# DecaYale/SYN3R

Measured on AMD Instinct MI355X. Metric: llff_3view_train_loop_iters_per_sec, higher is better.
Workload: dtype f32 raster / f16 UNet (f32 accumulate); 1 GPU; LLFF fern-like 3-view block: 50 raster fwd+bwd iters (l1 loss) (200000 Gaussians, 1920x1080, SH3) + 1 SVD (step,pass): CFG UNet fwd [2,14,8,72,128] f16 + fused Euler step; frames=14, parallelism=scene-parallel x1

## Files before the change

### include/syn3r_hip.h

```cpp
#ifndef SYN3R_HIP_H
#define SYN3R_HIP_H

#include <stddef.h>
#include <stdint.h>

#ifdef __cplusplus
extern "C" {
#endif

#define SYN3R_OK 0
#define SYN3R_E_INVALID (-1)
#define SYN3R_E_WORKSPACE (-2)
#define SYN3R_E_HIP (-3)

#define SYN3R_F32 0
#define SYN3R_F16 1

const char* syn3r_last_error(void);
int syn3r_version(void);
const char* syn3r_arch(void);

int syn3r_trace_enable(int on);
void* syn3r_trace_session(void);
int syn3r_trace_attach(void* session);
// ... 109 lines not shown
                                int W, int* radii, void* geom, size_t geom_bytes, long long* num_rendered_host,
                                int raw, int flags, const float* filter3d, void* stream);
int syn3r_raster_backward_f3d(int N, int sh_degree, int sh_coeffs, long long P, const float* means3D,
                              const float* scales, const float* rotations, const float* opacities, const float* shs,
                              const float* confidence, float scale_modifier, const float* viewmatrix,
                              const float* projmatrix, const float* campos, float tanfovx, float tanfovy, int H, int W,
                              const float* bg, const int* radii, void* geom, size_t geom_bytes,
                              const unsigned* point_list, void* image, size_t image_bytes, const float* dL_dcolor,
                              const float* dL_ddepth, const float* dL_dalpha, float* dL_dmeans3D, float* dL_dscales,
                              float* dL_drotations, float* dL_dopacities, float* dL_dshs, float* dL_dmeans2D,
                              float* dL_dconfidence, void* workspace, size_t workspace_bytes, int raw, int flags,
                              const float* filter3d, void* stream);
int syn3r_raster_backward_abs(int N, int sh_degree, int sh_coeffs, long long P, const float* means3D,
                              const float* scales, const float* rotations, const float* opacities, const float* shs,
                              const float* confidence, float scale_modifier, const float* viewmatrix,
                              const float* projmatrix, const float* campos, float tanfovx, float tanfovy, int H, int W,
                              const float* bg, const int* radii, void* geom, size_t geom_bytes,
                              const unsigned* point_list, void* image, size_t image_bytes, const float* dL_dcolor,
                              const float* dL_ddepth, const float* dL_dalpha, float* dL_dmeans3D, float* dL_dscales,
                              float* dL_drotations, float* dL_dopacities, float* dL_dshs, float* dL_dmeans2D,
                              float* dL_dconfidence, void* workspace, size_t workspace_bytes, int raw, int flags,
                              const float* filter3d, float* dL_dmeans2D_abs, void* stream);
size_t syn3r_raster_backward_cam_workspace_bytes(int N);
int syn3r_raster_backward_cam(int N, int sh_degree, int sh_coeffs, long long P, const float* means3D,
                              const float* scales, const float* rotations, const float* opacities, const float* shs,
                              const float* confidence, float scale_modifier, const float* viewmatrix,
                              const float* projmatrix, const float* campos, float tanfovx, float tanfovy, int H, int W,
                              const float* bg, const int* radii, void* geom, size_t geom_bytes,
                              const unsigned* point_list, void* image, size_t image_bytes, const float* dL_dcolor,
                              const float* dL_ddepth, const float* dL_dalpha, float* dL_dmeans3D, float* dL_dscales,
                              float* dL_drotations, float* dL_dopacities, float* dL_dshs, float* dL_dmeans2D,
                              float* dL_dconfidence, void* workspace, size_t workspace_bytes, int raw, int flags,
                              const float* filter3d, float* dL_dmeans2D_abs, float* dL_dcamera, int accumulate,
                              void* stream);

size_t syn3r_sort_pairs_workspace_bytes(long long n);
int syn3r_sort_pairs(unsigned long long* keys, unsigned* vals, unsigned long long* keys_tmp, unsigned* vals_tmp,
                     long long n, int nbits, void* workspace, size_t workspace_bytes, int* result_in_tmp,
                     void* stream);


int syn3r_gemm_f16(const void* A, long long lda, const void* W, void* out, long long ldc, const void* bias,
                   const void* rowvec, long long ldrv, int rows_per_vec, int rv_group_rows, const void* residual, long long ldr,
                   const void* aux, long long ldaux, float s_acc, float s_res, float s_aux, int M, int N, int K,
                   void* gn_partials, size_t gn_partials_bytes, int* gn_written, void* stream);

int syn3r_gemm_2src_supported(int M, int N, int K1, int K2, long long lda1, long long lda2);
int syn3r_gemm_2src_f16(const void* A1, long long lda1, int K1, const void* A2, long long lda2, int K2, const void* W,
                        void* out, long long ldc, const void* bias, int M, int N, void* gn_partials, size_t gn_partials_bytes,
                        int* gn_written, void* stream);

int syn3r_gemm_set_tile(int bm);

int syn3r_gemm_set_splitk_workspace(void* workspace, size_t bytes);

int syn3r_gemm_geglu_f16(const void* A, long long lda, const void* Wpacked, const void* bias_packed, void* out,
                         long long ldc, int M, int D, int K, void* stream);

size_t syn3r_feedforward_workspace_bytes(int M, int D);
int syn3r_feedforward_f16(const void* x, long long ldx, const void* w1_packed, const void* b1_packed, int D,
                          const void* w2, const void* b2, void* out, long long ldc, const void* residual,
                          long long ldr, const void* aux, long long ldaux, float s_acc, float s_res, float s_aux,
                          int M, int C_in, int C_out, void* workspace, size_t workspace_bytes, void* stream);

int syn3r_feedforward_p64_supported(int M, int D, int C_in);
int syn3r_feedforward_p64_f16(const void* x, long long ldx, const void* w1_packed64, const void* b1_packed64, int D,
                              const void* w2, const void* b2, void* out, long long ldc, const void* residual,
                              long long ldr, const void* aux, long long ldaux, float s_acc, float s_res, float s_aux,
                              int M, int C_in, int C_out, void* workspace, size_t workspace_bytes, void* stream);

int syn3r_feedforward_fused_f16(const void* x, long long ldx, const void* w1_chunked, const void* b1_chunked, int D,
                                const void* w2, const void* b2, void* out, long long ldc, const void* residual,
                                long long ldr, const void* aux, long long ldaux, float s_acc, float s_res, float s_aux,
                                int M, int C, void* stream);

int syn3r_feedforward_fused_ln_f16(const void* x, long long ldx, const void* ln_gamma, const void* ln_beta, float ln_eps,
                                   const void* w1_chunked, const void* b1_chunked, int D, const void* w2, const void* b2,
                                   void* out, long long ldc, const void* residual, long long ldr, const void* aux,
                                   long long ldaux, float s_acc, float s_res, float s_aux, int M, int C, void* stream);

int syn3r_feedforward_fused_addln_f16(const void* x, long long ldx, const void* addvec, int rows_per_vec, const void* ln_gamma,
                                      const void* ln_beta, float ln_eps, const void* w1_chunked, const void* b1_chunked, int D,
                                      const void* w2, const void* b2, void* out, long long ldc, const void* aux, long long ldaux,
                                      float s_acc, float s_res, float s_aux, int M, int C, void* stream);

int syn3r_layernorm_linear320_f16(const void* x, long long ldx, const void* ln_gamma, const void* ln_beta, float ln_eps,
                                  const void* W, void* out, long long ldc, int M, int N, int C, void* stream);

int syn3r_conv2d3x3_f16(const void* X, const void* W, void* out, long long ldc, const void* bias,
                        const void* rowvec, long long ldrv, int rows_per_vec, const void* residual, long long ldr,
                        float s_acc, float s_res, int NB, int Hi, int Wi, int Cin, int Cout, int stride, int upsample,
                        int pad_lo, void* gn_partials, size_t gn_partials_bytes, int* gn_written, void* stream);

int syn3r_pack_upsample4_f16(const void* w, void* w4, int Cout, int Cin);
int syn3r_conv2d3x3_up4_f16(const void* X, const void* w4, void* out, const void* bias, const void* residual, int NB, int Hi, int Wi,
                            int Cin, int Cout, void* gn_partials, size_t gn_partials_bytes, int* gn_written, void* stream);

int syn3r_tconv3_f16(const void* X, const void* W, void* out, long long ldc, const void* bias, const void* rowvec,
                     long long ldrv, int rows_per_vec, const void* residual, long long ldr, float s_acc, float s_res,
                     int B, int F, int HW, int Cin, int Cout, void* gn_partials, size_t gn_partials_bytes, int* gn_written,
                     void* stream);

int syn3r_attention_f16(const void* q, const void* k, const void* v, long long ld, void* out, long long ldo,
                        int nseq, int S, int heads, void* stream);

int syn3r_attention_temporal_f16(const void* q, const void* k, const void* v, long long ld, void* out,
// ... 161 lines not shown
```

### syn3r_amd/_lib.py

```python
from __future__ import annotations

import ctypes as C
from pathlib import Path

import torch

_LIB_PATH = Path(__file__).resolve().parent / "lib" / "libsyn3r_hip.so"
_lib = None

c_f = C.c_float
c_i = C.c_int
c_p = C.c_void_p
c_sz = C.c_size_t
c_ll = C.c_longlong
c_d = C.c_double

F32, F16 = 0, 1
RASTER_ANTIALIAS = 1

FILTER3D_VARIANCE, FILTER3D_NEAR, FILTER3D_MARGIN = 0.2, 0.2, 0.15

_SCENE = [c_p, c_p, c_p, c_p, c_p, c_p, c_f, c_p, c_p, c_p, c_f, c_f, c_i, c_i]
_RASTER_PREPROCESS = [c_i, c_i, c_i] + _SCENE + [c_p, c_p, c_sz, C.POINTER(c_ll)]
_RASTER_BACKWARD = ([c_i, c_i, c_i, c_ll] + _SCENE + [c_p, c_p, c_p, c_sz, c_p, c_p, c_sz]
# ... 2 lines not shown
_CAM = [c_i, c_i, c_p, c_p, c_p, c_i, c_p]
CAMERA_GRAD = 35

SIGNATURES = {
    "syn3r_last_error": (C.c_char_p, []),
    "syn3r_version": (c_i, []),
    "syn3r_arch": (C.c_char_p, []),
    "syn3r_trace_enable": (c_i, [c_i]),
    "syn3r_trace_filter": (c_i, [C.c_char_p]),
    "syn3r_trace_report": (c_i, [C.c_char_p, c_sz]),
    "syn3r_trace_session": (c_p, []),
    "syn3r_trace_attach": (c_i, [c_p]),
    "syn3r_inverse_warp_workspace_bytes": (c_sz, [c_i]),
    "syn3r_inverse_warp": (c_i, [c_p, c_p, c_p, c_p, c_p, c_p, c_p, c_f, c_i, c_i, c_i,
                                 c_p, c_p, c_p, c_p, c_p, c_p, c_p, c_p, c_p, c_p, c_p, c_p, c_sz, c_p]),
    "syn3r_reproj_error": (c_i, [c_p, c_p, c_p, c_p, c_p, c_p, c_p, c_i, c_i, c_p, c_p]),
    "syn3r_warp_post": (c_i, [c_p, c_p, c_p, c_i, c_i, c_i, c_i, c_i, c_p, c_p, c_p, c_p, c_p, c_p, c_p]),
    "syn3r_fuse_uncertainty": (c_i, [c_p, c_p, c_p, c_i, c_i, c_i, c_i, c_i, c_p, c_p, c_p, c_p]),
    "syn3r_forward_warp_workspace_bytes": (c_sz, [c_i, c_i]),
    "syn3r_forward_warp": (c_i, [c_p, c_p, c_p, c_p, c_p, c_p, c_i, c_i, c_p, c_p, c_p, c_p, c_sz, c_p]),
    "syn3r_step_workspace_bytes": (c_sz, [c_i, c_i, c_i, c_i]),
    "syn3r_step_interp": (c_i, [c_p, c_i, c_p, c_i, c_p, c_p, c_p, c_f, c_f, c_f, c_f, c_f, c_f, c_i,
                                c_p, c_p, c_p, c_i, c_i, c_i, c_i, c_p, c_sz, c_p]),
    "syn3r_step_replace": (c_i, [c_p, c_i, c_p, c_i, c_p, c_p, c_p, c_f, c_f, c_f, c_f,
                                 c_p, c_p, c_i, c_i, c_i, c_i, c_p, c_sz, c_p]),
    "syn3r_raster_geom_bytes": (c_sz, [c_i]),
    "syn3r_raster_image_bytes": (c_sz, [c_i, c_i]),
    "syn3r_raster_binning_bytes": (c_sz, [c_ll]),
    "syn3r_raster_preprocess": (c_i, _RASTER_PREPROCESS + _STREAM),
    "syn3r_raster_preprocess_raw": (c_i, _RASTER_PREPROCESS + _STREAM),
    "syn3r_raster_preprocess_ex": (c_i, _RASTER_PREPROCESS + _EX),
    "syn3r_raster_preprocess_f3d": (c_i, _RASTER_PREPROCESS + _F3D),
    "syn3r_raster_render": (c_i, [c_i, c_i, c_i, c_p, c_p, c_p, c_sz, c_p, c_sz, c_p, c_sz, c_ll, c_p, c_p, c_p,
                                  C.POINTER(c_p), c_p]),
    "syn3r_raster_backward_workspace_bytes": (c_sz, [c_i]),
    "syn3r_raster_backward": (c_i, _RASTER_BACKWARD + _STREAM),
    "syn3r_raster_backward_raw": (c_i, _RASTER_BACKWARD + _STREAM),
    "syn3r_raster_backward_ex": (c_i, _RASTER_BACKWARD + _EX),
    "syn3r_raster_backward_f3d": (c_i, _RASTER_BACKWARD + _F3D),
    "syn3r_raster_backward_abs": (c_i, _RASTER_BACKWARD + _ABS),
    "syn3r_raster_backward_cam_workspace_bytes": (c_sz, [c_i]),
    "syn3r_raster_backward_cam": (c_i, _RASTER_BACKWARD + _CAM),
    "syn3r_filter3d_workspace_bytes": (c_sz, [c_i]),
    "syn3r_filter3d_compute": (c_i, [c_p, c_i, c_p, c_i, c_f, c_f, c_f, c_p, c_p, c_sz, c_p]),
    "syn3r_sort_pairs_workspace_bytes": (c_sz, [c_ll]),
    "syn3r_sort_pairs": (c_i, [c_p, c_p, c_p, c_p, c_ll, c_i, c_p, c_sz, C.POINTER(c_i), c_p]),
    "syn3r_gaussian_activate": (c_i, [c_i, c_p, c_p, c_p, c_p, c_p, c_p, c_p]),
    "syn3r_gaussian_activate_backward": (c_i, [c_i, c_p, c_p, c_p, c_p, c_p, c_p, c_p, c_p, c_p, c_p, c_p]),
    "syn3r_densification_stats": (c_i, [c_i, c_p, c_p, c_p, c_p, c_p, c_p]),
    "syn3r_densification_stats_abs": (c_i, [c_i, c_p, c_p, c_p, c_p, c_p, c_p, c_p, c_p]),
    "syn3r_gemm_f16": (c_i, [c_p, c_ll, c_p, c_p, c_ll, c_p, c_p, c_ll, c_i, c_i, c_p, c_ll, c_p, c_ll, c_f, c_f, c_f,
                             c_i, c_i, c_i, c_p, c_sz, C.POINTER(c_i), c_p]),
    "syn3r_gemm_set_tile": (c_i, [c_i]),
    "syn3r_gemm_geglu_f16": (c_i, [c_p, c_ll, c_p, c_p, c_p, c_ll, c_i, c_i, c_i, c_p]),
    "syn3r_feedforward_workspace_bytes": (c_sz, [c_i, c_i]),
    "syn3r_feedforward_f16": (c_i, [c_p, c_ll, c_p, c_p, c_i, c_p, c_p, c_p, c_ll, c_p, c_ll, c_p, c_ll, c_f, c_f, c_f,
                                    c_i, c_i, c_i, c_p, c_sz, c_p]),
    "syn3r_feedforward_p64_f16": (c_i, [c_p, c_ll, c_p, c_p, c_i, c_p, c_p, c_p, c_ll, c_p, c_ll, c_p, c_ll, c_f, c_f, c_f,
                                    c_i, c_i, c_i, c_p, c_sz, c_p]),
    "syn3r_feedforward_p64_supported": (c_i, [c_i, c_i, c_i]),
    "syn3r_feedforward_fused_f16": (c_i, [c_p, c_ll, c_p, c_p, c_i, c_p, c_p, c_p, c_ll, c_p, c_ll, c_p, c_ll, c_f, c_f, c_f,
                                          c_i, c_i, c_p]),
    "syn3r_feedforward_fused_ln_f16": (c_i, [c_p, c_ll, c_p, c_p, c_f, c_p, c_p, c_i, c_p, c_p, c_p, c_ll, c_p, c_ll, c_p, c_ll,
                                             c_f, c_f, c_f, c_i, c_i, c_p]),
    "syn3r_feedforward_fused_addln_f16": (c_i, [c_p, c_ll, c_p, c_i, c_p, c_p, c_f, c_p, c_p, c_i, c_p, c_p, c_p, c_ll, c_p, c_ll,
                                                c_f, c_f, c_f, c_i, c_i, c_p]),
    "syn3r_layernorm_linear320_f16": (c_i, [c_p, c_ll, c_p, c_p, c_f, c_p, c_p, c_ll, c_i, c_i, c_i, c_p]),
    "syn3r_conv2d3x3_f16": (c_i, [c_p, c_p, c_p, c_ll, c_p, c_p, c_ll, c_i, c_p, c_ll, c_f, c_f,
                                  c_i, c_i, c_i, c_i, c_i, c_i, c_i, c_i, c_p, c_sz, C.POINTER(c_i), c_p]),
    "syn3r_pack_upsample4_f16": (c_i, [c_p, c_p, c_i, c_i]),
    "syn3r_conv2d3x3_up4_f16": (c_i, [c_p, c_p, c_p, c_p, c_p, c_i, c_i, c_i, c_i, c_i, c_p, c_sz, C.POINTER(c_i), c_p]),
    "syn3r_tconv3_f16": (c_i, [c_p, c_p, c_p, c_ll, c_p, c_p, c_ll, c_i, c_p, c_ll, c_f, c_f,
                               c_i, c_i, c_i, c_i, c_i, c_p, c_sz, C.POINTER(c_i), c_p]),
    "syn3r_attention_f16": (c_i, [c_p, c_p, c_p, c_ll, c_p, c_ll, c_i, c_i, c_i, c_p]),
    "syn3r_attention_temporal_f16": (c_i, [c_p, c_p, c_p, c_ll, c_p, c_ll, c_i, c_i, c_i, c_i, c_p]),
    "syn3r_groupnorm_workspace_bytes": (c_sz, [c_i, c_i]),
    "syn3r_groupnorm_f16": (c_i, [c_p, c_p, c_i, c_i, c_i, c_p, c_p, c_f, c_i, c_p, c_sz, c_p]),
    "syn3r_groupnorm_2src_f16": (c_i, [c_p, c_i, c_p, c_i, c_p, c_i, c_i, c_p, c_p, c_f, c_i, c_p, c_sz, c_p]),
    "syn3r_groupnorm_pre_f16": (c_i, [c_p, c_i, c_p, c_p, c_i, c_p, c_p, c_i, c_i, c_p, c_p, c_f, c_i, c_p, c_sz, c_p]),
    "syn3r_gn_partials_bytes": (c_sz, [c_i, c_i]),
    "syn3r_gemm_2src_supported": (c_i, [c_i, c_i, c_i, c_i, c_ll, c_ll]),
    "syn3r_gemm_2src_f16": (c_i, [c_p, c_ll, c_i, c_p, c_ll, c_i, c_p, c_p, c_ll, c_p, c_i, c_i, c_p, c_sz, C.POINTER(c_i), c_p]),
    "syn3r_layernorm_f16": (c_i, [c_p, c_p, c_p, c_p, c_i, c_ll, c_i, c_p, c_p, c_f, c_p]),
    "syn3r_geglu_f16": (c_i, [c_p, c_p, c_ll, c_i, c_p]),
    "syn3r_softmax_rows_f16": (c_i, [c_p, c_p, c_ll, c_i, c_ll, c_f, c_p]),
    "syn3r_time_conv_out": (c_i, [c_p, c_ll, c_p, c_p, c_p, c_i, c_i, c_ll, c_p]),
    "syn3r_l1_loss_workspace_bytes": (c_sz, [c_ll]),
    "syn3r_l1_loss": (c_i, [c_p, c_p, c_ll, c_f, c_p, c_p, c_sz, c_p]),
    "syn3r_l1_loss_backward": (c_i, [c_p, c_p, c_ll, c_f, c_p, c_p, c_p]),
    "syn3r_image_mse": (c_i, [c_p, c_p, c_ll, c_p, c_p, c_sz, c_p]),
    "syn3r_photo_loss_workspace_bytes": (c_sz, [c_i, c_i, c_i]),
    "syn3r_photo_loss": (c_i, [c_p, c_p, c_i, c_i, c_i, c_f, c_f, c_p, c_p, c_sz, c_p]),
    "syn3r_photo_loss_backward": (c_i, [c_p, c_p, c_i, c_i, c_i, c_f, c_f, c_p, c_p, c_p, c_p]),
    "syn3r_photo_loss_step": (c_i, [c_p, c_p, c_i, c_i, c_i, c_f, c_f, c_p, c_p, c_p, c_p, c_sz, c_p]),
    "syn3r_photo_loss_map_workspace_bytes": (c_sz, [c_i, c_i, c_i]),
    "syn3r_photo_loss_map": (c_i, [c_p, c_p, c_p, c_i, c_i, c_i, c_f, c_f, c_p, c_p, c_sz, c_p]),
    "syn3r_photo_loss_map_backward": (c_i, [c_p, c_p, c_p, c_i, c_i, c_i, c_f, c_f, c_p, c_p, c_p, c_p]),
    "syn3r_photo_loss_map_step": (c_i, [c_p, c_p, c_p, c_i, c_i, c_i, c_f, c_f, c_p, c_p, c_p, c_p, c_sz, c_p]),
    "syn3r_l1_loss_map": (c_i, [c_p, c_p, c_p, c_ll, c_ll, c_f, c_p, c_p, c_sz, c_p]),
    "syn3r_l1_loss_map_backward": (c_i, [c_p, c_p, c_p, c_ll, c_ll, c_f, c_p, c_p, c_p]),
    "syn3r_depth_corr_loss_workspace_bytes": (c_sz, [c_ll]),
    "syn3r_depth_corr_loss": (c_i, [c_p, c_p, c_ll, c_f, c_f, c_i, c_p, c_p, c_sz, c_p]),
    "syn3r_depth_corr_loss_backward": (c_i, [c_p, c_p, c_ll, c_f, c_f, c_i, c_p, c_p, c_sz, c_p, c_p]),
    "syn3r_depth_corr_loss_step": (c_i, [c_p, c_p, c_ll, c_f, c_f, c_i, c_p, c_p, c_p, c_p, c_sz, c_p]),
    "syn3r_exposure_apply": (c_i, [c_p, c_p, c_i, c_i, c_p, c_p]),
    "syn3r_exposure_backward_workspace_bytes": (c_sz, [c_i, c_i]),
# ... 174 lines not shown
```

### syn3r_amd/csrc/gemm.hip

```cpp
#include "common.h"
#include <cstdlib>
#include <algorithm>
#include <atomic>
#include <type_traits>

using namespace syn3r;

namespace {

#include "gemm_common.h"
#include "gemm_dma160.h"
#include "gemm_dma.h"
#include "gemm_wide.h"
#include "gemm_z.h"
#include "gemm_dmap.h"
#include "gemm_dmapd.h"
#include "gemm_g256.h"
#include "gemm_ffn.h"

int persistent_blocks() {
    static std::atomic<int> cus_of[64];
    static const int forced = tune_env("SYN3R_PERSISTENT_BLOCKS", 0);
    if (forced > 0) return forced < 8 ? 8 : forced;
    int dev = 0;
    if (hipGetDevice(&dev) != hipSuccess || dev < 0 || dev >= 64) dev = 0;
    int n = cus_of[dev].load(std::memory_order_relaxed);
    if (n == 0) {
        int v = 0;
        n = (hipDeviceGetAttribute(&v, hipDeviceAttributeMultiprocessorCount, dev) == hipSuccess && v > 0) ? v : 256;
        if (n < 8) n = 8;
        cus_of[dev].store(n, std::memory_order_relaxed);
    }
    return n;
}

size_t gn_partials_bytes(long long M, long long N) { return (size_t)(M / 32) * 2 * (size_t)(N / 10) * sizeof(float); }
int gn_request(GemmParams& p, void* buf, size_t bytes, const char* who) {
    SYN3R_REQUIRE((buf == nullptr) == (bytes == 0), "%s: gn_partials pointer and size must both be given or both be zero", who);
    SYN3R_REQUIRE(((uintptr_t)buf % 16) == 0, "%s: the gn_partials buffer must be 16-byte aligned", who);
    if (!buf || p.M % 32 != 0 || p.N % 80 != 0 || p.geglu_D > 0 || p.out_tiled || bytes < gn_partials_bytes(p.M, p.N)) return SYN3R_OK;
    p.gn_part = (float*)buf; p.gn_units = p.N / 10;
    return SYN3R_OK;
}

template <void (*KERNEL)(GemmParams)>
int launch_tiles(const char* family, size_t lds, long long grid, int block, hipStream_t stream, const GemmParams& q, int* gn_written,
                 const char* base, int b0 = 0, int b1 = 0) {
    static DevOnce once;
    if (int rc = set_max_lds(once, (const void*)KERNEL, (int)lds, family)) return rc;
    char name[96];
    if (trace_on()) {
        const int n = snprintf(name, sizeof(name), base, b0, b1);
        if (trace_detail()) snprintf(name + n, sizeof(name) - n, "[M%d,N%d,K%d,e%d]", q.M, q.N, q.K, q.geglu_D > 0 ? 2 : (q.residual != nullptr));
    }
    SYN3R_LAUNCH_NAMED(name, KERNEL, dim3((unsigned)grid), dim3(block), lds, stream, q);
    hipError_t e = hipGetLastError();
    if (e != hipSuccess) { set_error("%s launch: %s", family, hipGetErrorString(e)); return SYN3R_E_HIP; }
    if (gn_written) *gn_written = q.gn_part != nullptr;
    return SYN3R_OK;
}

long long wide_tiles(const GemmParams& p) { return (long long)((p.M + WBM - 1) / WBM) * ((p.N + WBN - 1) / WBN); }
bool wide_fills(const GemmParams& p) {
    const long long tiles = wide_tiles(p), rounds = (tiles + 255) / 256;
    return tiles * 10 >= rounds * 256 * 8;
}

int band_width(const GemmParams& p) {
    static const int band_env = tune_env("SYN3R_Z_BAND", 0);
    if (band_env > 0) return band_env;
// ... 155 lines not shown
    bool split = false;
    int rc = launch_splitk<MODE>(p, stream, &split);
    if (split || rc) return rc;
    int bm = g_dma_bm > 0 ? g_dma_bm : ((MODE != MODE_DENSE || tiles256(p) >= 256) ? 256 : 128);
    return bm == 128 ? launch_dma_bm<MODE, 128>(p, stream, gn_written) : launch_dma_bm<MODE, 256>(p, stream, gn_written);
}

int check_common(const GemmParams& p, const char* who) {
    SYN3R_REQUIRE(p.A && p.W && p.out, "%s: null operand", who);
    SYN3R_REQUIRE(SYN3R_DIM_OK(p.M) && SYN3R_DIM_OK(p.N) && SYN3R_DIM_OK(p.K), "%s: bad sizes M=%d N=%d K=%d", who, p.M, p.N, p.K);
    SYN3R_REQUIRE(p.K % BK == 0, "%s: K=%d must be a multiple of %d", who, p.K, BK);
    SYN3R_REQUIRE(p.ldc % 8 == 0 && p.ldc >= p.N, "%s: ldc=%lld must be >= N and a multiple of 8", who, p.ldc);
    SYN3R_REQUIRE(!p.residual || (p.ldr % 8 == 0 && p.ldr >= p.N), "%s: bad residual stride", who);
    SYN3R_REQUIRE(!p.aux || (p.ldaux % 8 == 0 && p.ldaux >= p.N), "%s: bad aux stride", who);
    SYN3R_REQUIRE(!p.rowvec || (p.rows_per_vec != 0 && p.ldrv >= p.N), "%s: bad rowvec arguments", who);
    SYN3R_REQUIRE(p.rv_group >= 0 && (p.rv_group == 0 || p.rows_per_vec < 0), "%s: rv_group_rows needs rows_per_vec < 0", who);
    SYN3R_REQUIRE(((uintptr_t)p.A | (uintptr_t)p.W | (uintptr_t)p.out | (uintptr_t)p.residual | (uintptr_t)p.aux) % 16 == 0,
                  "%s: operands must be 16-byte aligned", who);
    return SYN3R_OK;
}

int ffn_workspace_check(const char* who, const void* workspace, size_t workspace_bytes, size_t need) {
    if (!workspace || workspace_bytes < need) {
        set_error("%s: workspace %zu < %zu", who, workspace_bytes, need);
        return SYN3R_E_WORKSPACE;
    }
    SYN3R_REQUIRE((uintptr_t)workspace % 16 == 0, "%s: workspace must be 16-byte aligned", who);
    return SYN3R_OK;
}
int ffn_net2(const char* who, const void* hidden_tiled, int D, const void* w2, const void* b2, void* out, long long ldc, const void* residual,
             long long ldr, const void* aux, long long ldaux, float s_acc, float s_res, float s_aux, int M, int C_out, hipStream_t stream) {
    GemmParams q{};
    q.A = (const __half*)hidden_tiled; q.lda = D; q.a_tiled = 1; q.W = (const __half*)w2; q.out = (__half*)out; q.ldc = ldc;
    q.bias = (const __half*)b2; q.residual = (const __half*)residual; q.ldr = ldr; q.aux = (const __half*)aux; q.ldaux = ldaux;
    q.s_acc = s_acc; q.s_res = s_res; q.s_aux = s_aux; q.M = M; q.N = C_out; q.K = D;
    int rc = check_common(q, who);
    if (rc) return rc;
    return launch_dma<MODE_DENSE>(q, stream);
}

}

extern "C" int syn3r_gemm_set_splitk_workspace(void* workspace, size_t bytes) {
    SYN3R_REQUIRE((workspace == nullptr) == (bytes == 0), "gemm_set_splitk_workspace: pointer and size must both be given or both be zero");
    SYN3R_REQUIRE(((uintptr_t)workspace % 16) == 0, "gemm_set_splitk_workspace: the workspace must be 16-byte aligned");
    g_splitk_ws = workspace;
    g_splitk_bytes = bytes;
    return SYN3R_OK;
}

extern "C" size_t syn3r_gn_partials_bytes(int M, int N) {
    if (!SYN3R_DIM_OK(M) || !SYN3R_DIM_OK(N) || M % 32 != 0 || N % 80 != 0) return 0;
    return gn_partials_bytes(M, N);
}

extern "C" int syn3r_gemm_set_tile(int bm) {
    SYN3R_REQUIRE(bm == 0 || bm == -128 || bm == -256 || bm == -320 || bm == -322, "gemm_set_tile: bm must be 0, -128, -256, -320 or -322");
    g_dma_bm = (bm == -128 || bm == -256) ? -bm : bm;
    return SYN3R_OK;
}

extern "C" int syn3r_gemm_2src_supported(int M, int N, int K1, int K2, long long lda1, long long lda2) {
    if (M < 8 || N < 8 || M % 8 || N % 8 || K1 <= 0 || K2 <= 0 || K1 % BK || K2 % BK) return 0;
    if ((long long)M * lda1 >= (1ll << 31) || (long long)M * lda2 >= (1ll << 31) || (long long)N * (K1 + K2) >= (1ll << 31)) return 0;
    return 1;
}

constexpr int SKINNY_MAX_M = 16;
template <int MR>
__global__ void __launch_bounds__(256) k_gemm_skinny(GemmParams p) {
    const int lane = threadIdx.x & 63, wv = threadIdx.x >> 6;
    const int n0 = (blockIdx.x * 4 + wv) * 2;
    if (n0 >= p.N) return;
    const bool two = n0 + 1 < p.N;
    const __half* w0 = p.W + (long long)n0 * p.K;
    const __half* w1 = p.W + (long long)(two ? n0 + 1 : n0) * p.K;
    float acc0[MR], acc1[MR];
#pragma unroll
    for (int m = 0; m < MR; ++m) { acc0[m] = 0.f; acc1[m] = 0.f; }
    for (int k = lane * 8; k < p.K; k += 512) {
        const half8 a = *(const half8*)(w0 + k), b = *(const half8*)(w1 + k);
#pragma unroll
        for (int m = 0; m < MR; ++m) {
            if (m < p.M) {
                const half8 x = *(const half8*)(p.A + (long long)m * p.lda + k);
#pragma unroll
                for (int e = 0; e < 8; ++e) {
                    acc0[m] += (float)x[e] * (float)a[e];
                    acc1[m] += (float)x[e] * (float)b[e];
                }
            }
        }
    }
#pragma unroll
    for (int m = 0; m < MR; ++m) {
        if (m < p.M) {
            float s0 = wave_sum(acc0[m]), s1 = wave_sum(acc1[m]);
            if (lane == 0) {
                float b0 = p.bias ? __half2float(p.bias[n0]) : 0.f;
                p.out[(long long)m * p.ldc + n0] = __float2half((s0 + b0) * p.s_acc);
                if (two) {
                    float b1 = p.bias ? __half2float(p.bias[n0 + 1]) : 0.f;
                    p.out[(long long)m * p.ldc + n0 + 1] = __float2half((s1 + b1) * p.s_acc);
                }
            }
        }
// ... 329 lines not shown
```

### syn3r_amd/csrc/gemm_ffn.h

```cpp

constexpr int F_C = 320, F_HC = 64, F_BM = 128;
constexpr int F_X_BYTES = F_BM * F_C * 2;
constexpr int F_SLOT = 160 * BK * 2;

struct FfnParams {
    GemmParams e;
    const __half* w1;
    const __half* b1;
    int D;
    const __half* ln_g;
    const __half* ln_b;
    float ln_eps;
    const __half* ln_add;
    int ln_add_rpv;
};

typedef _Float16 half4v __attribute__((ext_vector_type(4)));
#define DS_READ64(dst, addr, OFF) asm volatile("ds_read_b64 %0, %1 offset:" #OFF : "=v"(dst) : "v"(addr))
#define DS_WRITE64(addr, val) asm volatile("ds_write_b64 %0, %1" ::"v"(addr), "v"(val) : "memory")

__device__ __forceinline__ void ln_tile320(char* smem_raw, int tid, int m0, int M, float cf, const __half* ln_g, const __half* ln_b,
                                           float ln_eps, const __half* add, int add_rpv) {
    {
        const int r = tid >> 2, part = tid & 3;
        const int f = (r >> 1) & 1;
        half8 xv[5][2], addv[5][2];
        if (add) {
            int m = m0 + r;
            m = m < M ? m : M - 1;
            const __half* av = add + (long long)(m / add_rpv) * F_C;
#pragma unroll
            for (int kt = 0; kt < 5; ++kt)
#pragma unroll
                for (int e = 0; e < 2; ++e) addv[kt][e] = *(const half8*)(av + (kt * 8 + part + 4 * (e ^ f)) * 8);
        }
        asm volatile("s_waitcnt vmcnt(0)" ::: "memory");
        __syncthreads();
#pragma unroll
        for (int kt = 0; kt < 5; ++kt)
#pragma unroll
            for (int e = 0; e < 2; ++e)
                xv[kt][e] = *(const half8*)(smem_raw + kt * 16384 + r * 128 + (((part + 4 * (e ^ f)) ^ (r & 7)) << 4));
        if (add) {
#pragma unroll
            for (int kt = 0; kt < 5; ++kt)
#pragma unroll
                for (int e = 0; e < 2; ++e) xv[kt][e] = xv[kt][e] + addv[kt][e];
        }
        float s0 = 0.f, s1 = 0.f;
#pragma unroll
        for (int kt = 0; kt < 5; ++kt)
#pragma unroll
            for (int i = 0; i < 8; ++i) { s0 += (float)xv[kt][0][i]; s1 += (float)xv[kt][1][i]; }
        const float sa = f ? s1 : s0, sb = f ? s0 : s1;
        float s = sa + sb;
        s += __shfl_xor(s, 2, 64);
        s += __shfl_xor(s, 1, 64);
        const float mean = s / cf;
        float q0 = 0.f, q1 = 0.f;
        {
#pragma clang fp contract(off)
#pragma unroll
            for (int kt = 0; kt < 5; ++kt)
#pragma unroll
                for (int i = 0; i < 8; ++i) {
                    const float da = (float)xv[kt][0][i] - mean, db = (float)xv[kt][1][i] - mean;
                    const float da2 = da * da, db2 = db * db;
                    q0 += da2; q1 += db2;
                }
        }
        const float qa = f ? q1 : q0, qb = f ? q0 : q1;
        float qq = qa + qb;
        qq += __shfl_xor(qq, 2, 64);
        qq += __shfl_xor(qq, 1, 64);
        const float rstd = rsqrtf(qq / cf + ln_eps);
#pragma unroll
        for (int kt = 0; kt < 5; ++kt)
#pragma unroll
            for (int e = 0; e < 2; ++e) {
                const int cv = kt * 8 + part + 4 * (e ^ f);
                const half8 g = *(const half8*)(ln_g + cv * 8), b = *(const half8*)(ln_b + cv * 8);
                half8 o;
#pragma unroll
                for (int i = 0; i < 8; ++i) o[i] = (_Float16)(((float)xv[kt][e][i] - mean) * rstd * (float)g[i] + (float)b[i]);
                *(half8*)(smem_raw + kt * 16384 + r * 128 + (((part + 4 * (e ^ f)) ^ (r & 7)) << 4)) = o;
            }
        __syncthreads();
    }

}

constexpr int R_SLOTS = 7;
constexpr int R_H = R_SLOTS * F_SLOT;
constexpr int R_BIAS = R_H + F_BM * F_HC * 2;
constexpr int R_LDS = R_BIAS + 8 * 512;

__global__ void __launch_bounds__(512, 2) k_ffn320r(FfnParams q) {
    const GemmParams& p = q.e;
    extern __shared__ __attribute__((aligned(16))) char smem_raw[];
    const int tid = threadIdx.x, lane = tid & 63;
    const int wv = __builtin_amdgcn_readfirstlane(tid >> 6);
    const int wm = wv >> 1, wn = wv & 1;
    const int tiles_m = (p.M + F_BM - 1) / F_BM;
    const int m0 = (int)xcd_remap(blockIdx.x, (unsigned)tiles_m) * F_BM;
    const int nchunks = q.D / F_HC;
    const long long D = q.D;
    const int fr = lane & 15, fq = lane >> 4;
    typedef _Float16 half4e __attribute__((ext_vector_type(4)));

    const int prow = lane >> 3;
    const int csrc = (lane & 7) ^ prow;
    const int nbw = wv < 4 ? 3 : 2;
    const int b_first = wv < 4 ? wv * 3 : 12 + (wv - 4) * 2;
    unsigned ow1 = (unsigned)((((wv * 2) * 8 + prow) * F_C + csrc * 8) * 2);
    unsigned ow2 = (unsigned)(((long long)(b_first * 8 + prow) * D + csrc * 8) * 2);
    unsigned ob1 = (unsigned)(lane * 4);
    char* const bias_line = smem_raw + R_BIAS + wv * 512;
    auto issue_w1 = [&](int ij, int ir) {
        asm volatile("" : "+v"(ow1), "+v"(ob1));
        long long soff = ((long long)ij * (128 * F_C) + ir * BK) * 2;
        asm volatile("" : "+s"(soff));
        const char* src = (const char*)q.w1 + soff;
        char* slot = smem_raw + ir * F_SLOT;
#pragma unroll
        for (int i = 0; i < 2; ++i)
            __builtin_amdgcn_global_load_lds((gbl_void_t*)(src + i * (8 * F_C * 2) + (size_t)ow1), (lds_void_t*)(slot + (wv * 2 + i) * 1024), 16, 0, 0);
        if (ir == 0) {
            long long boff = (long long)ij * 256;
            asm volatile("" : "+s"(boff));
            __builtin_amdgcn_global_load_lds((gbl_void_t*)((const char*)q.b1 + boff + (size_t)ob1), (lds_void_t*)(bias_line + (ij & 1) * 256), 4, 0, 0);
        }
    };
    auto issue_w2 = [&](int ij) {
        asm volatile("" : "+v"(ow2));
#pragma unroll
        for (int hh = 0; hh < 2; ++hh) {
            long long soff = ((long long)hh * 160 * D + (long long)ij * F_HC) * 2;
            asm volatile("" : "+s"(soff));
            const char* src = (const char*)p.W + soff;
            char* slot = smem_raw + (5 + hh) * F_SLOT;
// ... 250 lines not shown
                    half8 rr = res[it];
                    if (p.res_add) rr = rr + radd[it];
#pragma unroll
                    for (int e = 0; e < 8; ++e) f[e] += p.s_res * (float)rr[e];
                }
                if (p.aux) {
                    const half8 av = *(const half8*)(p.aux + (long long)m * p.ldaux + n);
#pragma unroll
                    for (int e = 0; e < 8; ++e) f[e] += p.s_aux * (float)av[e];
                }
#pragma unroll
                for (int e = 0; e < 8; ++e) v[e] = (_Float16)f[e];
            }
            *(half8*)(p.out + (long long)m * p.ldc + n) = v;
        }
    }
}

int launch_ffn320(const FfnParams& q, hipStream_t stream) {
    static DevOnce once;
    int rc = set_max_lds(once, (const void*)k_ffn320r, R_LDS, "hipFuncSetAttribute(ffn320r)");
    if (rc) return rc;
    const int tiles = (q.e.M + F_BM - 1) / F_BM;
    char name[96];
    if (trace_on()) {
        if (trace_detail()) snprintf(name, sizeof(name), "k_gemm_ffn320[M%d,D%d,e%d]", q.e.M, q.D, q.e.residual != nullptr);
        else snprintf(name, sizeof(name), "k_gemm_ffn320");
    }
    SYN3R_LAUNCH_NAMED(name, k_ffn320r, dim3(tiles), dim3(512), R_LDS, stream, q);
    SYN3R_LAUNCH_CHECK("ffn320r launch");
    return SYN3R_OK;
}

constexpr int Q_SLOT = F_C * 32 * 2;
constexpr int Q_RING = F_X_BYTES;
constexpr int Q_ST = Q_RING + 3 * Q_SLOT;
constexpr int Q_ST_WAVE = 16 * WN * 2;
constexpr int Q_LDS = Q_ST + 8 * Q_ST_WAVE;

struct LnLinParams {
    const __half* x; long long ldx;
    const __half* W;
    __half* out; long long ldc;
    int M, N, C;
    const __half* ln_g; const __half* ln_b; float ln_eps;
};

__global__ void __launch_bounds__(512, 2) k_lnlin320(LnLinParams p) {
    extern __shared__ __attribute__((aligned(16))) char smem_raw[];
    const int tid = threadIdx.x, lane = tid & 63;
    const int wv = __builtin_amdgcn_readfirstlane(tid >> 6);
    const int wm = wv >> 2, wn = wv & 3;
    const int tiles_m = (p.M + F_BM - 1) / F_BM;
    const int m0 = (int)xcd_remap(blockIdx.x, (unsigned)tiles_m) * F_BM;
    const int nstage = (p.N / F_C) * 10;
    const bool full = m0 + F_BM <= p.M;

    const int wprow = lane >> 2;
    const int wcsrc = (lane & 3) ^ h_swz(wprow);
    const int nbw = wv < 4 ? 3 : 2;
    const int b_first = wv < 4 ? wv * 3 : 12 + (wv - 4) * 2;
    const __half* w_lane = p.W + (long long)(b_first * 16 + wprow) * F_C + wcsrc * 8;
    char* const ring = smem_raw + Q_RING;
    int ig = 0, islot = 0;
    auto issue_next = [&]() {
        if (ig >= nstage) return;
        const int c = ig / 10, ks = ig - c * 10;
        const __half* src = w_lane + (long long)c * (F_C * F_C) + ks * 32;
        char* slot = ring + islot * Q_SLOT;
#pragma unroll
        for (int i = 0; i < 3; ++i)
            if (i < nbw)
                __builtin_amdgcn_global_load_lds((gbl_void_t*)(src + i * 16 * F_C), (lds_void_t*)(slot + (b_first + i) * 1024), 16, 0, 0);
        ++ig;
        if (++islot == 3) islot = 0;
    };

    {
        const int prow = lane >> 3;
        const int csrc = (lane & 7) ^ prow;
#pragma unroll
        for (int kt = 0; kt < 5; ++kt)
#pragma unroll
            for (int i = 0; i < 2; ++i) {
                int m = m0 + (wv * 2 + i) * 8 + prow;
                m = m < p.M ? m : p.M - 1;
                __builtin_amdgcn_global_load_lds((gbl_void_t*)(p.x + (long long)m * p.ldx + kt * BK + csrc * 8),
                                                 (lds_void_t*)(smem_raw + kt * 16384 + (wv * 2 + i) * 1024), 16, 0, 0);
            }
    }
    issue_next();
    issue_next();
    ln_tile320(smem_raw, tid, m0, p.M, (float)p.C, p.ln_g, p.ln_b, p.ln_eps, nullptr, 1);

    const int fr = lane & 15, fq = lane >> 4;
    const unsigned lds0 = (unsigned)(size_t)(__attribute__((address_space(3))) char*)smem_raw;
    const unsigned sw0 = (unsigned)(((0 + fq) ^ (fr & 7)) << 4), sw1 = (unsigned)(((4 + fq) ^ (fr & 7)) << 4);
    const unsigned x_row = lds0 + (unsigned)((wm * 64 + fr) * 128);
    const unsigned w_row = (unsigned)((wn * 80 + fr) * 64) + (unsigned)((fq ^ h_swz(fr)) << 4);
    const unsigned st_base = lds0 + Q_ST + (unsigned)(wv * Q_ST_WAVE);
    unsigned st_wr[TN];
#pragma unroll
    for (int j = 0; j < TN; ++j) st_wr[j] = st_base + (unsigned)(fr * (WN * 2) + ((j * 2 + (fq >> 1) + fr) % 10) * 16 + (fq & 1) * 8);
    int st_col[3];
#pragma unroll
    for (int it = 0; it < 3; ++it) {
        const int q = lane + it * 64, row = q / (WN / 8), chp = q - row * (WN / 8);
        st_col[it] = ((chp + 20 - row) % 10) * 8;
    }
    typedef _Float16 half4e __attribute__((ext_vector_type(4)));

    int cslot = 0, g = 0;
    const int nchunks = p.N / F_C;
    for (int c = 0; c < nchunks; ++c) {
        float4v acc[TM][TN];
#pragma unroll
        for (int i = 0; i < TM; ++i)
#pragma unroll
            for (int j = 0; j < TN; ++j) acc[i][j] = (float4v){0.f, 0.f, 0.f, 0.f};
#pragma unroll
        for (int ks = 0; ks < 10; ++ks, ++g) {
            if (g + 1 >= nstage) asm volatile("s_waitcnt vmcnt(0)" ::: "memory");
            else if (ks < 2 && c > 0 && full) {
                if (wv < 4) asm volatile("s_waitcnt vmcnt(15)" ::: "memory");
                else asm volatile("s_waitcnt vmcnt(14)" ::: "memory");
            } else {
                if (wv < 4) asm volatile("s_waitcnt vmcnt(3)" ::: "memory");
                else asm volatile("s_waitcnt vmcnt(2)" ::: "memory");
            }
            __builtin_amdgcn_s_barrier();
            const unsigned xa = x_row + (unsigned)((ks >> 1) * 16384) + ((ks & 1) ? sw1 : sw0);
            const unsigned wa = lds0 + Q_RING + (unsigned)(cslot * Q_SLOT) + w_row;
            half8 a[TM], b[TN];
            DS_READ128(a[0], xa, 0); DS_READ128(a[1], xa, 2048); DS_READ128(a[2], xa, 4096); DS_READ128(a[3], xa, 6144);
            DS_READ128(b[0], wa, 0); DS_READ128(b[1], wa, 1024); DS_READ128(b[2], wa, 2048); DS_READ128(b[3], wa, 3072);
            DS_READ128(b[4], wa, 4096);
            issue_next();
            asm volatile("s_waitcnt lgkmcnt(4)" : "+v"(a[0]), "+v"(a[1]), "+v"(a[2]), "+v"(a[3]), "+v"(b[0]));
#pragma unroll
            for (int i = 0; i < TM; ++i) acc[i][0] = __builtin_amdgcn_mfma_f32_16x16x32_f16(b[0], a[i], acc[i][0], 0, 0, 0);
            __builtin_amdgcn_sched_barrier(0);
            asm volatile("s_waitcnt lgkmcnt(3)" : "+v"(b[1]));
#pragma unroll
            for (int i = 0; i < TM; ++i) acc[i][1] = __builtin_amdgcn_mfma_f32_16x16x32_f16(b[1], a[i], acc[i][1], 0, 0, 0);
            __builtin_amdgcn_sched_barrier(0);
            asm volatile("s_waitcnt lgkmcnt(2)" : "+v"(b[2]));
#pragma unroll
            for (int i = 0; i < TM; ++i) acc[i][2] = __builtin_amdgcn_mfma_f32_16x16x32_f16(b[2], a[i], acc[i][2], 0, 0, 0);
            __builtin_amdgcn_sched_barrier(0);
            asm volatile("s_waitcnt lgkmcnt(1)" : "+v"(b[3]));
#pragma unroll
            for (int i = 0; i < TM; ++i) acc[i][3] = __builtin_amdgcn_mfma_f32_16x16x32_f16(b[3], a[i], acc[i][3], 0, 0, 0);
            __builtin_amdgcn_sched_barrier(0);
            asm volatile("s_waitcnt lgkmcnt(0)" : "+v"(b[4]));
#pragma unroll
            for (int i = 0; i < TM; ++i) acc[i][4] = __builtin_amdgcn_mfma_f32_16x16x32_f16(b[4], a[i], acc[i][4], 0, 0, 0);
            __builtin_amdgcn_sched_barrier(0);
            if (++cslot == 3) cslot = 0;
        }
        __half* const orow = p.out + (long long)c * F_C + wn * WN;
#pragma unroll
        for (int i = 0; i < TM; ++i) {
#pragma unroll
            for (int j = 0; j < TN; ++j) {
                half4e o;
#pragma unroll
                for (int r = 0; r < 4; ++r) o[r] = (_Float16)acc[i][j][r];
                DS_WRITE64(st_wr[j], o);
            }
            asm volatile("s_waitcnt lgkmcnt(0)" ::: "memory");
            __builtin_amdgcn_wave_barrier();
            half8 v[3];
            DS_READ128(v[0], st_base + (unsigned)(lane * 16), 0);
            DS_READ128(v[1], st_base + (unsigned)(lane * 16), 1024);
            DS_READ128(v[2], st_base + (unsigned)((lane & 31) * 16), 2048);
            asm volatile("s_waitcnt lgkmcnt(0)" : "+v"(v[0]), "+v"(v[1]), "+v"(v[2]));
            __builtin_amdgcn_wave_barrier();
#pragma unroll
            for (int it = 0; it < 3; ++it) {
                const int q = lane + it * 64;
                const int row = q / (WN / 8);
                const int m = m0 + wm * WM + i * 16 + row;
                if (q < 16 * (WN / 8) && m < p.M) *(half8*)(orow + (long long)m * p.ldc + st_col[it]) = v[it];
            }
        }
    }
}

int launch_lnlin320(const LnLinParams& p, hipStream_t stream) {
    static DevOnce once;
    if (int rc = set_max_lds(once, (const void*)k_lnlin320, (int)(Q_LDS), "hipFuncSetAttribute(lnlin320)")) return rc;
    const int tiles = (p.M + F_BM - 1) / F_BM;
    char name[96];
    if (trace_on()) {
        if (trace_detail()) snprintf(name, sizeof(name), "k_gemm_lnlin320[M%d,N%d]", p.M, p.N);
        else snprintf(name, sizeof(name), "k_gemm_lnlin320");
    }
    SYN3R_LAUNCH_NAMED(name, k_lnlin320, dim3(tiles), dim3(512), Q_LDS, stream, p);
    SYN3R_LAUNCH_CHECK("lnlin320 launch");
    return SYN3R_OK;
}
```

Before: 416.6 iters/s.

## Make lnlin320 GEMM persistent with next-tile X prefetch and continuous weight ring

Converts the layernorm+linear320 kernel to a persistent grid capped at the device's block count, with XCD-aware tile assignment. Each block loops over several M-tiles, prefetching the next tile's X rows into LDS during the last chunk and letting the weight ring keep streaming across tiles. It also relaxes the vmcnt waits so stores can stay in flight. This targets launch tail and the prologue load latency, at the cost of more complex waitcnt accounting that is easy to get subtly wrong. A new API allows overriding the block count.

```diff
diff --git a/include/syn3r_hip.h b/include/syn3r_hip.h
--- a/include/syn3r_hip.h
+++ b/include/syn3r_hip.h
@@ -185,6 +185,8 @@
 
 int syn3r_gemm_set_tile(int bm);
 
+int syn3r_gemm_set_persistent_blocks(int n);
+
 int syn3r_gemm_set_splitk_workspace(void* workspace, size_t bytes);
 
 int syn3r_gemm_geglu_f16(const void* A, long long lda, const void* Wpacked, const void* bias_packed, void* out,
diff --git a/syn3r_amd/_lib.py b/syn3r_amd/_lib.py
--- a/syn3r_amd/_lib.py
+++ b/syn3r_amd/_lib.py
@@ -78,6 +78,7 @@
     "syn3r_gemm_f16": (c_i, [c_p, c_ll, c_p, c_p, c_ll, c_p, c_p, c_ll, c_i, c_i, c_p, c_ll, c_p, c_ll, c_f, c_f, c_f,
                              c_i, c_i, c_i, c_p, c_sz, C.POINTER(c_i), c_p]),
     "syn3r_gemm_set_tile": (c_i, [c_i]),
+    "syn3r_gemm_set_persistent_blocks": (c_i, [c_i]),
     "syn3r_gemm_geglu_f16": (c_i, [c_p, c_ll, c_p, c_p, c_p, c_ll, c_i, c_i, c_i, c_p]),
     "syn3r_feedforward_workspace_bytes": (c_sz, [c_i, c_i]),
     "syn3r_feedforward_f16": (c_i, [c_p, c_ll, c_p, c_p, c_i, c_p, c_p, c_p, c_ll, c_p, c_ll, c_p, c_ll, c_f, c_f, c_f,
diff --git a/syn3r_amd/csrc/gemm.hip b/syn3r_amd/csrc/gemm.hip
--- a/syn3r_amd/csrc/gemm.hip
+++ b/syn3r_amd/csrc/gemm.hip
@@ -16,6 +16,8 @@
 #include "gemm_dmap.h"
 #include "gemm_dmapd.h"
 #include "gemm_g256.h"
+int persistent_blocks();
+thread_local int g_level0_blocks = 0;
 #include "gemm_ffn.h"
 
 int persistent_blocks() {
@@ -277,6 +279,12 @@
 extern "C" size_t syn3r_gn_partials_bytes(int M, int N) {
     if (!SYN3R_DIM_OK(M) || !SYN3R_DIM_OK(N) || M % 32 != 0 || N % 80 != 0) return 0;
     return gn_partials_bytes(M, N);
+}
+
+extern "C" int syn3r_gemm_set_persistent_blocks(int n) {
+    SYN3R_REQUIRE(n >= 0, "gemm_set_persistent_blocks: n must be >= 1 (force the grid) or 0 (by device)");
+    g_level0_blocks = n;
+    return SYN3R_OK;
 }
 
 extern "C" int syn3r_gemm_set_tile(int bm) {
diff --git a/syn3r_amd/csrc/gemm_ffn.h b/syn3r_amd/csrc/gemm_ffn.h
--- a/syn3r_amd/csrc/gemm_ffn.h
+++ b/syn3r_amd/csrc/gemm_ffn.h
@@ -2,6 +2,17 @@
 constexpr int F_C = 320, F_HC = 64, F_BM = 128;
 constexpr int F_X_BYTES = F_BM * F_C * 2;
 constexpr int F_SLOT = 160 * BK * 2;
+
+int level0_grid(int tiles) { return std::min(tiles, g_level0_blocks > 0 ? g_level0_blocks : persistent_blocks()); }
+__device__ __forceinline__ XcdTiles level0_tiles(unsigned nblk) {
+    const unsigned nx = gridDim.x < 8 ? gridDim.x : 8;
+    const unsigned xcd = blockIdx.x % 8, q = nblk / nx, r = nblk % nx;
+    XcdTiles t;
+    t.start = xcd < r ? xcd * (q + 1) : r * (q + 1) + (xcd - r) * q;
+    t.len = q + (xcd < r ? 1u : 0u);
+    t.stride = (gridDim.x - xcd + 7) / 8;
+    return t;
+}
 
 struct FfnParams {
     GemmParams e;
@@ -20,7 +31,7 @@
 #define DS_WRITE64(addr, val) asm volatile("ds_write_b64 %0, %1" ::"v"(addr), "v"(val) : "memory")
 
 __device__ __forceinline__ void ln_tile320(char* smem_raw, int tid, int m0, int M, float cf, const __half* ln_g, const __half* ln_b,
-                                           float ln_eps, const __half* add, int add_rpv) {
+                                           float ln_eps, const __half* add, int add_rpv, bool stores_behind = false) {
     {
         const int r = tid >> 2, part = tid & 3;
         const int f = (r >> 1) & 1;
@@ -34,8 +45,9 @@
 #pragma unroll
                 for (int e = 0; e < 2; ++e) addv[kt][e] = *(const half8*)(av + (kt * 8 + part + 4 * (e ^ f)) * 8);
         }
-        asm volatile("s_waitcnt vmcnt(0)" ::: "memory");
-        __syncthreads();
+        if (stores_behind && !add) asm volatile("s_waitcnt vmcnt(12)" ::: "memory");
+        else asm volatile("s_waitcnt vmcnt(0)" ::: "memory");
+        __builtin_amdgcn_s_barrier();
 #pragma unroll
         for (int kt = 0; kt < 5; ++kt)
 #pragma unroll
@@ -85,7 +97,8 @@
                 for (int i = 0; i < 8; ++i) o[i] = (_Float16)(((float)xv[kt][e][i] - mean) * rstd * (float)g[i] + (float)b[i]);
                 *(half8*)(smem_raw + kt * 16384 + r * 128 + (((part + 4 * (e ^ f)) ^ (r & 7)) << 4)) = o;
             }
-        __syncthreads();
+        asm volatile("s_waitcnt lgkmcnt(0)" ::: "memory");
+        __builtin_amdgcn_s_barrier();
     }
 
 }
@@ -442,9 +455,10 @@
     const int wv = __builtin_amdgcn_readfirstlane(tid >> 6);
     const int wm = wv >> 2, wn = wv & 3;
     const int tiles_m = (p.M + F_BM - 1) / F_BM;
-    const int m0 = (int)xcd_remap(blockIdx.x, (unsigned)tiles_m) * F_BM;
+    const XcdTiles tiles = level0_tiles((unsigned)tiles_m);
+    unsigned pos = blockIdx.x / 8;
+    if (pos >= tiles.len) return;
     const int nstage = (p.N / F_C) * 10;
-    const bool full = m0 + F_BM <= p.M;
 
     const int wprow = lane >> 2;
     const int wcsrc = (lane & 3) ^ h_swz(wprow);
@@ -452,9 +466,13 @@
     const int b_first = wv < 4 ? wv * 3 : 12 + (wv - 4) * 2;
     const __half* w_lane = p.W + (long long)(b_first * 16 + wprow) * F_C + wcsrc * 8;
     char* const ring = smem_raw + Q_RING;
+    bool has_next = pos + tiles.stride < tiles.len;
     int ig = 0, islot = 0;
     auto issue_next = [&]() {
-        if (ig >= nstage) return;
+        if (ig >= nstage) {
+            if (!has_next) return;
+            ig = 0;
+        }
         const int c = ig / 10, ks = ig - c * 10;
         const __half* src = w_lane + (long long)c * (F_C * F_C) + ks * 32;
         char* slot = ring + islot * Q_SLOT;
@@ -466,22 +484,25 @@
         if (++islot == 3) islot = 0;
     };
 
+    const int xprow = lane >> 3;
+    const int xcsrc = (lane & 7) ^ xprow;
+    auto issue_x = [&](int mx, int kt) {
+#pragma unroll
+        for (int i = 0; i < 2; ++i) {
+            int m = mx + (wv * 2 + i) * 8 + xprow;
+            m = m < p.M ? m : p.M - 1;
+            __builtin_amdgcn_global_load_lds((gbl_void_t*)(p.x + (long long)m * p.ldx + kt * BK + xcsrc * 8),
+                                             (lds_void_t*)(smem_raw + kt * 16384 + (wv * 2 + i) * 1024), 16, 0, 0);
+        }
+    };
+
     {
-        const int prow = lane >> 3;
-        const int csrc = (lane & 7) ^ prow;
-#pragma unroll
-        for (int kt = 0; kt < 5; ++kt)
-#pragma unroll
-            for (int i = 0; i < 2; ++i) {
-                int m = m0 + (wv * 2 + i) * 8 + prow;
-                m = m < p.M ? m : p.M - 1;
-                __builtin_amdgcn_global_load_lds((gbl_void_t*)(p.x + (long long)m * p.ldx + kt * BK + csrc * 8),
-                                                 (lds_void_t*)(smem_raw + kt * 16384 + (wv * 2 + i) * 1024), 16, 0, 0);
-            }
+        const int m_first = (int)(tiles.start + pos) * F_BM;
+#pragma unroll
+        for (int kt = 0; kt < 5; ++kt) issue_x(m_first, kt);
     }
     issue_next();
     issue_next();
-    ln_tile320(smem_raw, tid, m0, p.M, (float)p.C, p.ln_g, p.ln_b, p.ln_eps, nullptr, 1);
 
     const int fr = lane & 15, fq = lane >> 4;
     const unsigned lds0 = (unsigned)(size_t)(__attribute__((address_space(3))) char*)smem_raw;
@@ -500,20 +521,35 @@
     }
     typedef _Float16 half4e __attribute__((ext_vector_type(4)));
 
-    int cslot = 0, g = 0;
+    int cslot = 0;
     const int nchunks = p.N / F_C;
+    bool stores_behind = false;
+    for (;; pos += tiles.stride) {
+    const int m0 = (int)(tiles.start + pos) * F_BM;
+    const int m_next = m0 + (int)tiles.stride * F_BM;
+    has_next = pos + tiles.stride < tiles.len;
+    const bool full = m0 + F_BM <= p.M;
+    const __half *ln_g = p.ln_g, *ln_b = p.ln_b;
+    asm volatile("" : "+s"(ln_g), "+s"(ln_b));
+    ln_tile320(smem_raw, tid, m0, p.M, (float)p.C, ln_g, ln_b, p.ln_eps, nullptr, 1, stores_behind);
     for (int c = 0; c < nchunks; ++c) {
         float4v acc[TM][TN];
 #pragma unroll
         for (int i = 0; i < TM; ++i)
 #pragma unroll
             for (int j = 0; j < TN; ++j) acc[i][j] = (float4v){0.f, 0.f, 0.f, 0.f};
-#pragma unroll
-        for (int ks = 0; ks < 10; ++ks, ++g) {
-            if (g + 1 >= nstage) asm volatile("s_waitcnt vmcnt(0)" ::: "memory");
-            else if (ks < 2 && c > 0 && full) {
-                if (wv < 4) asm volatile("s_waitcnt vmcnt(15)" ::: "memory");
+        const bool xpre = has_next && c + 1 == nchunks;
+#pragma unroll
+        for (int ks = 0; ks < 10; ++ks) {
+            if (c == 0 && ks < 2) {
+            } else if (ks == 9 && c + 1 == nchunks && !has_next) asm volatile("s_waitcnt vmcnt(0)" ::: "memory");
+            else if (ks < 2) {
+                if (!full) asm volatile("s_waitcnt vmcnt(0)" ::: "memory");
+                else if (wv < 4) asm volatile("s_waitcnt vmcnt(15)" ::: "memory");
                 else asm volatile("s_waitcnt vmcnt(14)" ::: "memory");
+            } else if (ks >= 3 && xpre) {
+                if (wv < 4) asm volatile("s_waitcnt vmcnt(5)" ::: "memory");
+                else asm volatile("s_waitcnt vmcnt(4)" ::: "memory");
             } else {
                 if (wv < 4) asm volatile("s_waitcnt vmcnt(3)" ::: "memory");
                 else asm volatile("s_waitcnt vmcnt(2)" ::: "memory");
@@ -526,6 +562,7 @@
             DS_READ128(b[0], wa, 0); DS_READ128(b[1], wa, 1024); DS_READ128(b[2], wa, 2048); DS_READ128(b[3], wa, 3072);
             DS_READ128(b[4], wa, 4096);
             issue_next();
+            if (xpre && ks >= 2 && (ks & 1) == 0) issue_x(m_next, (ks >> 1) - 1);
             asm volatile("s_waitcnt lgkmcnt(4)" : "+v"(a[0]), "+v"(a[1]), "+v"(a[2]), "+v"(a[3]), "+v"(b[0]));
 #pragma unroll
             for (int i = 0; i < TM; ++i) acc[i][0] = __builtin_amdgcn_mfma_f32_16x16x32_f16(b[0], a[i], acc[i][0], 0, 0, 0);
@@ -547,6 +584,10 @@
             for (int i = 0; i < TM; ++i) acc[i][4] = __builtin_amdgcn_mfma_f32_16x16x32_f16(b[4], a[i], acc[i][4], 0, 0, 0);
             __builtin_amdgcn_sched_barrier(0);
             if (++cslot == 3) cslot = 0;
+        }
+        if (xpre) {
+            __builtin_amdgcn_s_barrier();
+            issue_x(m_next, 4);
         }
         __half* const orow = p.out + (long long)c * F_C + wn * WN;
 #pragma unroll
@@ -575,6 +616,9 @@
             }
         }
     }
+    if (!has_next) break;
+    stores_behind = full;
+    }
 }
 
 int launch_lnlin320(const LnLinParams& p, hipStream_t stream) {
@@ -586,7 +630,7 @@
         if (trace_detail()) snprintf(name, sizeof(name), "k_gemm_lnlin320[M%d,N%d]", p.M, p.N);
         else snprintf(name, sizeof(name), "k_gemm_lnlin320");
     }
-    SYN3R_LAUNCH_NAMED(name, k_lnlin320, dim3(tiles), dim3(512), Q_LDS, stream, p);
+    SYN3R_LAUNCH_NAMED(name, k_lnlin320, dim3(level0_grid(tiles)), dim3(512), Q_LDS, stream, p);
     SYN3R_LAUNCH_CHECK("lnlin320 launch");
     return SYN3R_OK;
 }
```

After: 415.9 iters/s, median of 2. About the same (-0.2%).
